# sidward14/gan-lab

Hardware: AMD Instinct MI355X
Metric: images/sec (G+D step), StyleGAN 1024^2 bs32/GPU (higher is better)
Workload: dtype f32; 1 GPU; StyleGAN res_samples=1024 FFHQ-shaped synthetic, bs=32/GPU fp32, nonsaturating + R1(lambda=10) + drift, stabilised phase, 1 D-iter + 1 G-iter; global_batch=32, per_gpu_batch=32, parallelism=single

## Files before the change

gan_lab_amd/csrc/conv_x3_wgrad.hip:

```cpp
#include "x3_common.h"

namespace {

constexpr int XW_CO = 32, XW_CI = 64;
constexpr int XW_GP = 7, XW_XP = 5;
constexpr int XW_GPL = XW_CO * XW_GP, XW_XPL = XW_CI * XW_XP;
constexpr int XW_GROW = 3 * XW_GPL;
constexpr int XW_XROW = 3 * XW_XPL;
constexpr int XW_XOFF = 2 * XW_GROW;
constexpr int XW_ZERO = 4;
constexpr int XW_LDS = 2 * XW_GROW + 5 * XW_XROW;
constexpr int XW_DUMP = 32;

#define XW_ACC9(a) "+v"(a[0]), "+v"(a[1]), "+v"(a[2]), "+v"(a[3]), "+v"(a[4]), "+v"(a[5]), "+v"(a[6]), "+v"(a[7]), "+v"(a[8])

struct XWArgs {
  const float* gy;
  const float* x;
  float* part;
  const float* aff_s;
  const float* aff_t;
  int N, CI, CO, H, W;
  int hshift;
  int strips_x, nstrips;
  int tiles_ci, splits, sps;
};

template <bool AFF>
__global__ __launch_bounds__(512) void conv_x3_wgrad_kernel(XWArgs p) {
  __shared__ __attribute__((aligned(16))) u32x4 lds[XW_LDS];
  const int tid = threadIdx.x, lane = tid & 63;
  const int wv = __builtin_amdgcn_readfirstlane(tid >> 6);
  const int wc = wv >> 2, wi = wv & 3;
  const int l16 = lane & 15, kg = lane >> 4;

  int b = blockIdx.x;
  const int split = b % p.splits; b /= p.splits;
  const int ci_t = b % p.tiles_ci;
  const int co_t = b / p.tiles_ci;
  const int co0 = co_t * XW_CO, ci0 = ci_t * XW_CI;
  const int s_first = split * p.sps;
  const int s_count = min(p.sps, p.nstrips - s_first);
  const int F = s_count << p.hshift;
  const int hmask = p.H - 1;
  const long long plane = (long long)p.H * p.W;

  const u32x4 rs_g = x3_rsrc(p.gy, (unsigned)((long long)p.N * p.CO * plane * 4));
  const u32x4 rs_x = x3_rsrc(p.x, (unsigned)((long long)p.N * p.CI * plane * 4));

  const bool g_item = tid < 320;
  const int g_co = g_item ? tid / 10 : 0, g_q = g_item ? tid % 10 : 0;
  const int g_dst = ((g_co * XW_GP + ((g_q + 1) >> 1)) * 16 + ((g_q + 1) & 1) * 8);
  const int x_ci = tid >> 3, x_q = tid & 7;
  const int x_dst = ((x_ci * XW_XP + (x_q >> 1)) * 16 + (x_q & 1) * 8);
  float a_s = 1.f, a_t = 0.f;
  int aff_n = -1;

  auto flat_pos = [&](int f, int& n, int& y, int& x0) {
    const int strip = s_first + (f >> p.hshift);
    y = f & hmask;
    n = strip / p.strips_x;
    x0 = (strip - n * p.strips_x) * 32;
  };
  auto g_off = [&](int f) {
    int n, y, x0;
    flat_pos(f, n, y, x0);
    const int px = x0 - 4 + 4 * g_q;
    const bool ok = g_item && f < F && px >= 0 && px < p.W;
    return ok ? (int)((((long long)n * p.CO + co0 + g_co) * plane + (long long)y * p.W + px) * 4) : (int)0x80000000;
  };
  auto x_off = [&](int f) {
    int n, y, x0;
    flat_pos(f, n, y, x0);
    return f < F ? (int)((((long long)n * p.CI + ci0 + x_ci) * plane + (long long)y * p.W + x0 + 4 * x_q) * 4) : (int)0x80000000;
  };
  auto g_store = [&](const f32x4& v, int buf) {
    if (!g_item) return;
    u32x2 h, m, l;
    x3_split4(v, h, m, l);
    unsigned char* d = reinterpret_cast<unsigned char*>(lds + buf * XW_GROW) + g_dst;
    *reinterpret_cast<u32x2*>(d) = h;
    *reinterpret_cast<u32x2*>(d + XW_GPL * 16) = m;
    *reinterpret_cast<u32x2*>(d + 2 * XW_GPL * 16) = l;
  };
  auto x_store = [&](f32x4 v, int slot, int f) {
    if constexpr (AFF) {
      int n, y, x0;
      flat_pos(f, n, y, x0);
      if (n != aff_n && f < F) {
        aff_n = n;
        a_s = p.aff_s[(long long)n * p.CI + ci0 + x_ci];
        a_t = p.aff_t[(long long)n * p.CI + ci0 + x_ci];
      }
#pragma unroll
      for (int j = 0; j < 4; ++j) v[j] = fmaf(v[j], a_s, a_t);
    }
    u32x2 h, m, l;
    x3_split4(v, h, m, l);
    unsigned char* d = reinterpret_cast<unsigned char*>(lds + XW_XOFF + slot * XW_XROW) + x_dst;
    *reinterpret_cast<u32x2*>(d) = h;
    *reinterpret_cast<u32x2*>(d + XW_XPL * 16) = m;
    *reinterpret_cast<u32x2*>(d + 2 * XW_XPL * 16) = l;
  };

  f32x4 accS[9], accH[9], accT[9];
#pragma unroll
  for (int t = 0; t < 9; ++t) { accS[t] = f32x4{0.f, 0.f, 0.f, 0.f}; accH[t] = f32x4{0.f, 0.f, 0.f, 0.f}; accT[t] = f32x4{0.f, 0.f, 0.f, 0.f}; }

  X3_SETTLE(XW_ACC9(accS));
  X3_SETTLE(XW_ACC9(accH));
  const int laneG = (wc * 16 + l16) * XW_GP + 1 + kg;
  const int laneX = XW_XOFF + (wi * 16 + l16) * XW_XP + kg;

  u32x4 gc[3];
  unsigned gp_[3], gn_[3];
  bf16x8 aS[3][3];
  bf16x8 bX[2][3];
  auto g_frags = [&](int buf) {
#pragma unroll
    for (int pl = 0; pl < 3; ++pl) {
      const int u = buf * XW_GROW + pl * XW_GPL + laneG;
      gc[pl] = lds[u];
      gp_[pl] = reinterpret_cast<const unsigned*>(lds + u - 1)[3];
      gn_[pl] = reinterpret_cast<const unsigned*>(lds + u + 1)[0];
    }
  };
  auto a_build = [&]() {
#pragma unroll
    for (int pl = 0; pl < 3; ++pl) {
      const u32x4 c = gc[pl];
      u32x4 up, dn;
      up[0] = __builtin_amdgcn_alignbit(c[1], c[0], 16); up[1] = __builtin_amdgcn_alignbit(c[2], c[1], 16);
      up[2] = __builtin_amdgcn_alignbit(c[3], c[2], 16); up[3] = __builtin_amdgcn_alignbit(gn_[pl], c[3], 16);
      dn[0] = __builtin_amdgcn_alignbit(c[0], gp_[pl], 16); dn[1] = __builtin_amdgcn_alignbit(c[1], c[0], 16);
      dn[2] = __builtin_amdgcn_alignbit(c[2], c[1], 16); dn[3] = __builtin_amdgcn_alignbit(c[3], c[2], 16);
      aS[0][pl] = __builtin_bit_cast(bf16x8, up);
      aS[1][pl] = __builtin_bit_cast(bf16x8, c);
      aS[2][pl] = __builtin_bit_cast(bf16x8, dn);
    }
  };
  auto x_frags = [&](int slot, int set) {
#pragma unroll
    for (int pl = 0; pl < 3; ++pl) bX[set][pl] = __builtin_bit_cast(bf16x8, lds[laneX + slot * XW_XROW + pl * XW_XPL]);
  };

  for (int i = tid; i < XW_XROW; i += 512) lds[XW_XOFF + XW_ZERO * XW_XROW + i] = u32x4{0u, 0u, 0u, 0u};
  f32x4 gA, xA, gB, xB;
  x3_ld(gA, rs_g, g_off(0)); x3_ld(xA, rs_x, x_off(0));
  x3_ld(gB, rs_g, (int)0x80000000); x3_ld(xB, rs_x, x_off(1));
  x3_ld_wait<0>(gA, xA);
  x3_ld_wait<0>(gB, xB);
  g_store(gA, 0); x_store(xA, 0, 0); x_store(xB, 1, 1);
  asm volatile("s_waitcnt lgkmcnt(0)\n\ts_barrier" ::: "memory");
  x3_ld(gA, rs_g, g_off(1)); x3_ld(xA, rs_x, x_off(2));
  x3_ld(gB, rs_g, g_off(2)); x3_ld(xB, rs_x, x_off(3));
  g_frags(0);
  x_frags(XW_ZERO, 0);

  int since_dump = 0;
  for (int f0 = 0; f0 < F; f0 += 4) {
#pragma unroll
    for (int u = 0; u < 4; ++u) {
      const int f = f0 + u;
      const int y = f & hmask;
      const int slot1 = u, slot2 = y == hmask ? XW_ZERO : (u + 1) & 3;
      a_build();
      __builtin_amdgcn_sched_barrier(0);
      x_frags(slot1, 1);
      __builtin_amdgcn_sched_barrier(0);
#pragma unroll
      for (int kx = 0; kx < 3; ++kx) {
        X3_MFMA(accS[kx], aS[kx][2], bX[0][0]); X3_MFMA(accS[kx], aS[kx][0], bX[0][2]); X3_MFMA(accS[kx], aS[kx][1], bX[0][1]);
        X3_MFMA(accS[kx], aS[kx][1], bX[0][0]); X3_MFMA(accS[kx], aS[kx][0], bX[0][1]); X3_MFMA(accH[kx], aS[kx][0], bX[0][0]);
      }
      __builtin_amdgcn_sched_barrier(0);
      if (u & 1) { x3_ld_wait<2>(gB, xB); g_store(gB, (u + 1) & 1); x_store(xB, (u + 2) & 3, f + 2); }
      else { x3_ld_wait<2>(gA, xA); g_store(gA, (u + 1) & 1); x_store(xA, (u + 2) & 3, f + 2); }
      __builtin_amdgcn_sched_barrier(0);
      x_frags(slot2, 0);
      __builtin_amdgcn_sched_barrier(0);
#pragma unroll
      for (int kx = 0; kx < 3; ++kx) {
        X3_MFMA(accS[3 + kx], aS[kx][2], bX[1][0]); X3_MFMA(accS[3 + kx], aS[kx][0], bX[1][2]); X3_MFMA(accS[3 + kx], aS[kx][1], bX[1][1]);
        X3_MFMA(accS[3 + kx], aS[kx][1], bX[1][0]); X3_MFMA(accS[3 + kx], aS[kx][0], bX[1][1]); X3_MFMA(accH[3 + kx], aS[kx][0], bX[1][0]);
      }
      __builtin_amdgcn_sched_barrier(0);
      if (u & 1) { x3_ld(gB, rs_g, g_off(f + 3)); x3_ld(xB, rs_x, x_off(f + 4)); }
      else { x3_ld(gA, rs_g, g_off(f + 3)); x3_ld(xA, rs_x, x_off(f + 4)); }
      asm volatile("s_waitcnt lgkmcnt(0)\n\ts_barrier" ::: "memory");
      __builtin_amdgcn_sched_barrier(0);
      g_frags((u + 1) & 1);
      __builtin_amdgcn_sched_barrier(0);
#pragma unroll
      for (int kx = 0; kx < 3; ++kx) {
        X3_MFMA(accS[6 + kx], aS[kx][2], bX[0][0]); X3_MFMA(accS[6 + kx], aS[kx][0], bX[0][2]); X3_MFMA(accS[6 + kx], aS[kx][1], bX[0][1]);
        X3_MFMA(accS[6 + kx], aS[kx][1], bX[0][0]); X3_MFMA(accS[6 + kx], aS[kx][0], bX[0][1]); X3_MFMA(accH[6 + kx], aS[kx][0], bX[0][0]);
      }
      __builtin_amdgcn_sched_barrier(0);
      x_frags(y == hmask ? XW_ZERO : u, 0);
      if (++since_dump == XW_DUMP) {
        since_dump = 0;
        X3_DRAIN(XW_ACC9(accH));
#pragma unroll
        for (int t = 0; t < 9; ++t) { accT[t] += accH[t]; accH[t] = f32x4{0.f, 0.f, 0.f, 0.f}; }
        X3_SETTLE(XW_ACC9(accH));
      }
      __builtin_amdgcn_sched_barrier(0);
    }
  }

  X3_DRAIN(XW_ACC9(accS));
  X3_DRAIN(XW_ACC9(accH));
  float* dst = p.part + (long long)split * p.CO * p.CI * 9;
#pragma unroll
  for (int t = 0; t < 9; ++t) {
    const f32x4 v = accT[t] + accH[t] + accS[t];
#pragma unroll
    for (int r = 0; r < 4; ++r)
      dst[((long long)(co0 + wc * 16 + 4 * kg + r) * p.CI + ci0 + wi * 16 + l16) * 9 + t] = v[r];
  }
}

__global__ void x3w_reduce_kernel(const float* __restrict__ part, float* __restrict__ out, long long n, int slots, float scale) {
  const long long i = blockIdx.x * (long long)blockDim.x + threadIdx.x;
  if (i >= n) return;
  float s0 = 0.f, s1 = 0.f, s2 = 0.f, s3 = 0.f;
  int k = 0;
  for (; k + 3 < slots; k += 4) {
    s0 += part[(long long)k * n + i]; s1 += part[(long long)(k + 1) * n + i];
    s2 += part[(long long)(k + 2) * n + i]; s3 += part[(long long)(k + 3) * n + i];
  }
  for (; k < slots; ++k) s0 += part[(long long)k * n + i];
  out[i] = ((s0 + s1) + (s2 + s3)) * scale;
}

struct XWPlan { int splits, sps; };
bool xw_ok(const ganlab_conv_geom* g) {
  if (g == nullptr || g->ks != 3 || g->pad != 1 || g->up || g->pool || g->N <= 0) return false;
  const int H = g->Hin, W = g->Win;
  if (H < 4 || (H & (H - 1)) != 0 || W % 32 != 0) return false;
  if (g->Cin % XW_CI != 0 || g->Cout % XW_CO != 0) return false;
  const long long bytes = (long long)g->N * (g->Cin > g->Cout ? g->Cin : g->Cout) * H * W * 4;
  return bytes < 0x7fffffffLL;
}
XWPlan xw_plan(const ganlab_conv_geom* g) {
  const int pairs = (g->Cout / XW_CO) * (g->Cin / XW_CI);
  const int nstrips = g->N * (g->Win / 32);
  int splits = (512 + pairs - 1) / pairs;
  if (splits > nstrips) splits = nstrips;
  if (splits < 1) splits = 1;
  const int sps = (nstrips + splits - 1) / splits;
  splits = (nstrips + sps - 1) / sps;
  return XWPlan{splits, sps};
}

}

extern "C" {

int ganlab_conv_wgrad_x3_supported(const ganlab_conv_geom* g) { return xw_ok(g) ? 1 : 0; }

size_t ganlab_conv_wgrad_x3_workspace(const ganlab_conv_geom* g) {
  if (!xw_ok(g)) return 0;
  return (size_t)xw_plan(g).splits * g->Cout * g->Cin * 9 * sizeof(float);
}

int ganlab_conv_wgrad_x3(const float* gy, const float* x, const float* aff_s, const float* aff_t, float* gw,
                         const ganlab_conv_geom* g, float scale, void* workspace, size_t workspace_bytes, void* stream) {
  if (!xw_ok(g)) return GANLAB_EUNSUPPORTED;
  if (!gy || !x || !gw || (aff_s == nullptr) != (aff_t == nullptr)) return GANLAB_EINVAL;
  const XWPlan pl = xw_plan(g);
  const long long nw = (long long)g->Cout * g->Cin * 9;
  if (!workspace || workspace_bytes < (size_t)pl.splits * nw * sizeof(float)) return GANLAB_EWORKSPACE;
  XWArgs a{};
  a.gy = gy; a.x = x; a.part = reinterpret_cast<float*>(workspace); a.aff_s = aff_s; a.aff_t = aff_t;
  a.N = g->N; a.CI = g->Cin; a.CO = g->Cout; a.H = g->Hin; a.W = g->Win;
  a.hshift = 0;
  while ((1 << a.hshift) < a.H) ++a.hshift;
  a.strips_x = a.W / 32; a.nstrips = a.N * a.strips_x;
  a.tiles_ci = a.CI / XW_CI; a.splits = pl.splits; a.sps = pl.sps;
  const long long grid = (long long)(a.CO / XW_CO) * a.tiles_ci * pl.splits;
  if (grid <= 0 || grid > 0x7fffffffLL) return GANLAB_EINVAL;
  hipStream_t st = gl_stream(stream);
  if (aff_s != nullptr) GL_LAUNCH(conv_x3_wgrad_kernel<true>, dim3((unsigned)grid), dim3(512), 0, st, a);
  else GL_LAUNCH(conv_x3_wgrad_kernel<false>, dim3((unsigned)grid), dim3(512), 0, st, a);
  GL_LAUNCH(x3w_reduce_kernel, dim3((unsigned)((nw + 255) / 256)), dim3(256), 0, st, (const float*)a.part, gw, nw, pl.splits, scale);
  return GL_CHECK_LAUNCH();
}

}
```

Measured before the change: 170.1 images/sec.

## Extend x3 wgrad kernel to 8x8 and 16x16 maps by packing images into strips

Lets the 3x3 weight-gradient kernel handle feature maps narrower than 32 columns (8x8 and 16x16) by packing several batch images side by side into one 32-wide strip. Halo words at image seams are masked to zero and out-of-range images are guarded. Low-resolution layers that previously fell back to a slower generic path can now use the fast bf16-split kernel. The seam masking and index remapping add some complexity, and if a seam were handled wrongly the gradients would be incorrect.

```diff
diff --git a/gan_lab_amd/csrc/conv_x3_wgrad.hip b/gan_lab_amd/csrc/conv_x3_wgrad.hip
--- a/gan_lab_amd/csrc/conv_x3_wgrad.hip
+++ b/gan_lab_amd/csrc/conv_x3_wgrad.hip
@@ -23,6 +23,7 @@
   int N, CI, CO, H, W;
   int hshift;
   int strips_x, nstrips;
+  int pack, wshift;
   int tiles_ci, splits, sps;
 };
 
@@ -56,23 +57,38 @@
   float a_s = 1.f, a_t = 0.f;
   int aff_n = -1;
 
+  const bool packed = p.pack > 1;
+  const int g_spx = 4 * g_q - 4;
+  const int g_sub = packed ? g_spx >> p.wshift : 0, g_col = packed ? g_spx & (p.W - 1) : 0;
+  const int x_sub = packed ? (4 * x_q) >> p.wshift : 0, x_col = packed ? (4 * x_q) & (p.W - 1) : 0;
   auto flat_pos = [&](int f, int& n, int& y, int& x0) {
     const int strip = s_first + (f >> p.hshift);
     y = f & hmask;
-    n = strip / p.strips_x;
-    x0 = (strip - n * p.strips_x) * 32;
+    const int q = strip / p.strips_x;
+    n = q * p.pack;
+    x0 = (strip - q * p.strips_x) * 32;
   };
   auto g_off = [&](int f) {
     int n, y, x0;
     flat_pos(f, n, y, x0);
-    const int px = x0 - 4 + 4 * g_q;
-    const bool ok = g_item && f < F && px >= 0 && px < p.W;
+    int px = x0 - 4 + 4 * g_q;
+    bool ok = g_item && f < F && px >= 0 && px < p.W;
+    if (packed) {
+      n += g_sub; px = g_col;
+      ok = g_item && f < F && g_spx >= 0 && g_spx < 32 && n < p.N;
+    }
     return ok ? (int)((((long long)n * p.CO + co0 + g_co) * plane + (long long)y * p.W + px) * 4) : (int)0x80000000;
   };
   auto x_off = [&](int f) {
     int n, y, x0;
     flat_pos(f, n, y, x0);
-    return f < F ? (int)((((long long)n * p.CI + ci0 + x_ci) * plane + (long long)y * p.W + x0 + 4 * x_q) * 4) : (int)0x80000000;
+    int px = x0 + 4 * x_q;
+    bool ok = f < F;
+    if (packed) {
+      n += x_sub; px = x_col;
+      ok = ok && n < p.N;
+    }
+    return ok ? (int)((((long long)n * p.CI + ci0 + x_ci) * plane + (long long)y * p.W + px) * 4) : (int)0x80000000;
   };
   auto g_store = [&](const f32x4& v, int buf) {
     if (!g_item) return;
@@ -87,10 +103,12 @@
     if constexpr (AFF) {
       int n, y, x0;
       flat_pos(f, n, y, x0);
+      n += x_sub;
       if (n != aff_n && f < F) {
         aff_n = n;
-        a_s = p.aff_s[(long long)n * p.CI + ci0 + x_ci];
-        a_t = p.aff_t[(long long)n * p.CI + ci0 + x_ci];
+        const bool in = n < p.N;
+        a_s = in ? p.aff_s[(long long)n * p.CI + ci0 + x_ci] : 0.f;
+        a_t = in ? p.aff_t[(long long)n * p.CI + ci0 + x_ci] : 0.f;
       }
 #pragma unroll
       for (int j = 0; j < 4; ++j) v[j] = fmaf(v[j], a_s, a_t);
@@ -111,6 +129,8 @@
   X3_SETTLE(XW_ACC9(accH));
   const int laneG = (wc * 16 + l16) * XW_GP + 1 + kg;
   const int laneX = XW_XOFF + (wi * 16 + l16) * XW_XP + kg;
+  const unsigned seam_p = packed && ((8 * kg) & (p.W - 1)) == 0 ? 0u : ~0u;
+  const unsigned seam_n = packed && ((8 * kg + 8) & (p.W - 1)) == 0 ? 0u : ~0u;
 
   u32x4 gc[3];
   unsigned gp_[3], gn_[3];
@@ -121,8 +141,8 @@
     for (int pl = 0; pl < 3; ++pl) {
       const int u = buf * XW_GROW + pl * XW_GPL + laneG;
       gc[pl] = lds[u];
-      gp_[pl] = reinterpret_cast<const unsigned*>(lds + u - 1)[3];
-      gn_[pl] = reinterpret_cast<const unsigned*>(lds + u + 1)[0];
+      gp_[pl] = reinterpret_cast<const unsigned*>(lds + u - 1)[3] & seam_p;
+      gn_[pl] = reinterpret_cast<const unsigned*>(lds + u + 1)[0] & seam_n;
     }
   };
   auto a_build = [&]() {
@@ -235,17 +255,26 @@
 }
 
 struct XWPlan { int splits, sps; };
+int xw_pack(int H, int W) {
+  if (W % 32 == 0) return 1;
+  if (H == W && (W == 16 || W == 8)) return 32 / W;
+  return 0;
+}
 bool xw_ok(const ganlab_conv_geom* g) {
   if (g == nullptr || g->ks != 3 || g->pad != 1 || g->up || g->pool || g->N <= 0) return false;
   const int H = g->Hin, W = g->Win;
-  if (H < 4 || (H & (H - 1)) != 0 || W % 32 != 0) return false;
+  if (H < 4 || (H & (H - 1)) != 0 || W <= 0 || xw_pack(H, W) == 0) return false;
   if (g->Cin % XW_CI != 0 || g->Cout % XW_CO != 0) return false;
   const long long bytes = (long long)g->N * (g->Cin > g->Cout ? g->Cin : g->Cout) * H * W * 4;
   return bytes < 0x7fffffffLL;
 }
+int xw_nstrips(const ganlab_conv_geom* g) {
+  const int pack = xw_pack(g->Hin, g->Win);
+  return pack > 1 ? (g->N + pack - 1) / pack : g->N * (g->Win / 32);
+}
 XWPlan xw_plan(const ganlab_conv_geom* g) {
   const int pairs = (g->Cout / XW_CO) * (g->Cin / XW_CI);
-  const int nstrips = g->N * (g->Win / 32);
+  const int nstrips = xw_nstrips(g);
   int splits = (512 + pairs - 1) / pairs;
   if (splits > nstrips) splits = nstrips;
   if (splits < 1) splits = 1;
@@ -277,7 +306,9 @@
   a.N = g->N; a.CI = g->Cin; a.CO = g->Cout; a.H = g->Hin; a.W = g->Win;
   a.hshift = 0;
   while ((1 << a.hshift) < a.H) ++a.hshift;
-  a.strips_x = a.W / 32; a.nstrips = a.N * a.strips_x;
+  a.pack = xw_pack(a.H, a.W);
+  a.wshift = a.W == 8 ? 3 : 4;
+  a.strips_x = a.pack > 1 ? 1 : a.W / 32; a.nstrips = xw_nstrips(g);
   a.tiles_ci = a.CI / XW_CI; a.splits = pl.splits; a.sps = pl.sps;
   const long long grid = (long long)(a.CO / XW_CO) * a.tiles_ci * pl.splits;
   if (grid <= 0 || grid > 0x7fffffffLL) return GANLAB_EINVAL;
```

Measured after the change: 171.0 images/sec, median of 6. No clear change (+0.6%).
